# quiver-team/torch-quiver

Measured on AMD Instinct MI355X. Metric: train-sampled-edges/sec (GraphSAGE e2e step, ogbn-products-shaped synthetic), higher is better.
Workload: dtype fp32; 1 GPU; model=graphsage-3L-h256 ogbn-products, global_batch=1024, parallelism=dp1, sample_mode=GPU, cache=196M, cache_policy=device_replicate, placement=degree, overlap=True

## Files before the change

### csrc/gather_kernels.hip

```cpp
#include <cstdlib>

#include "qk_common.h"

namespace qk {

namespace {

constexpr int BLOCK = 256;

struct alignas(16) vec16 { uint64_t a, b; };

template <typename VecT, int SUB, bool SCATTER>
__global__ void __launch_bounds__(BLOCK)
copy_rows_kernel(GatherSpec spec, const int64_t* __restrict__ indices,
                 int64_t n, char* __restrict__ other,
                 const int64_t* __restrict__ n_dev,
                 const int64_t* __restrict__ order, int64_t order_n) {
    if (n_dev) n = min(n, *n_dev);
    const int sub_id = threadIdx.x / SUB;
    const int lane = threadIdx.x % SUB;
    const int rows_per_block = BLOCK / SUB;
    int64_t row = (int64_t)blockIdx.x * rows_per_block + sub_id;
    const int64_t stride = (int64_t)gridDim.x * rows_per_block;
    const int64_t nvec = spec.row_bytes / (int64_t)sizeof(VecT);

    for (; row < n; row += stride) {
        int64_t idx = indices[row];
        if (order) {
            if (idx < 0 || idx >= order_n) continue;
            idx = order[idx];
        }
        if (idx < 0) continue;
        int s = 0;
        while (s < spec.nshards && idx >= spec.ends[s]) ++s;
        if (s >= spec.nshards) continue;
        if (!((spec.access_mask >> s) & 1u)) continue;
        const int64_t start = (s == 0) ? 0 : spec.ends[s - 1];
        const char* shard_row =
            spec.ptrs[s] + (idx - start) * spec.row_bytes;
        char* io_row = other + row * spec.row_bytes;
        if (SCATTER) {
            VecT* dst = (VecT*)shard_row;
            const VecT* src = (const VecT*)io_row;
            for (int64_t j = lane; j < nvec; j += SUB) dst[j] = src[j];
        } else {
            const VecT* src = (const VecT*)shard_row;
            VecT* dst = (VecT*)io_row;
            for (int64_t j = lane; j < nvec; j += SUB) dst[j] = src[j];
        }
    }
}

inline int grid_for(int64_t work, int per_block, int max_blocks) {
    int64_t blocks = (work + per_block - 1) / per_block;
    if (blocks > max_blocks) blocks = max_blocks;
    if (blocks < 1) blocks = 1;
    return (int)blocks;
}

inline int gather_max_blocks(const GatherSpec& spec, bool overlapped) {
    static int env_cap = [] {
        const char* e = getenv("QUIVER_GATHER_BLOCKS");
        return e ? atoi(e) : 0;
    }();
    if (env_cap > 0) return env_cap;
    if (!spec.has_host_shard) return 2048;
    if (overlapped) return spec.row_bytes <= 256 ? 160 : 112;
    return 640;
}

template <typename VecT, bool SCATTER>
void dispatch_sub(hipStream_t s, const GatherSpec& spec,
                  const int64_t* indices, int64_t n, char* other,
                  const int64_t* n_dev, const int64_t* order,
                  int64_t order_n) {
    int64_t nvec = spec.row_bytes / (int64_t)sizeof(VecT);
    int sub = 4;
    while (sub < 64 && sub < nvec) sub *= 2;
    int grid = grid_for(n, BLOCK / sub,
                        gather_max_blocks(spec, n_dev != nullptr));
    switch (sub) {
#define QK_CASE(S)                                                          \
    case S:                                                                 \
        copy_rows_kernel<VecT, S, SCATTER><<<grid, BLOCK, 0, s>>>(          \
            spec, indices, n, other, n_dev, order, order_n);                \
        break;
        QK_CASE(4) QK_CASE(8) QK_CASE(16) QK_CASE(32) QK_CASE(64)
#undef QK_CASE
    }
    QK_CHECK_HIP(hipGetLastError());
}

template <bool SCATTER>
void copy_rows(hipStream_t s, const GatherSpec& spec, const int64_t* indices,
               int64_t n, char* other, const int64_t* n_dev,
               const int64_t* order, int64_t order_n) {
    if (n == 0 || spec.nshards == 0) return;
    if (spec.row_bytes % 16 == 0)
        dispatch_sub<vec16, SCATTER>(s, spec, indices, n, other, n_dev,
                                     order, order_n);
    else if (spec.row_bytes % 8 == 0)
        dispatch_sub<uint64_t, SCATTER>(s, spec, indices, n, other, n_dev,
                                        order, order_n);
    else if (spec.row_bytes % 4 == 0)
        dispatch_sub<uint32_t, SCATTER>(s, spec, indices, n, other, n_dev,
                                        order, order_n);
    else
        dispatch_sub<uint8_t, SCATTER>(s, spec, indices, n, other, n_dev,
                                       order, order_n);
}

}

void launch_gather(hipStream_t s, const GatherSpec& spec,
                   const int64_t* indices, int64_t n, char* out,
                   const int64_t* n_dev, const int64_t* order,
                   int64_t order_n) {
    copy_rows<false>(s, spec, indices, n, out, n_dev, order, order_n);
}

void launch_scatter(hipStream_t s, const GatherSpec& spec,
                    const int64_t* indices, int64_t n, const char* src) {
    copy_rows<true>(s, spec, indices, n, const_cast<char*>(src), nullptr,
                    nullptr, 0);
}

}
```

### csrc/module.cpp

```cpp
#include <torch/extension.h>

#include <ATen/Parallel.h>
#include <c10/hip/HIPCachingAllocator.h>
#include <c10/hip/HIPStream.h>
#include <hip/hip_runtime.h>
#include <rccl/rccl.h>

#include <algorithm>
#include <atomic>
#include <condition_variable>
#include <functional>
#include <mutex>
#include <thread>
#include <random>
#include <unordered_map>
#include <vector>

#include "qk_common.h"

namespace {

#define QK_CHECK_RCCL(expr)                                                   \
    do {                                                                      \
        ncclResult_t _r = (expr);                                             \
        if (_r != ncclSuccess) {                                              \
            throw std::runtime_error(std::string("RCCL error: ") +            \
                                     ncclGetErrorString(_r));                 \
        }                                                                     \
    } while (0)

inline hipStream_t current_stream() {
    return c10::hip::getCurrentHIPStream().stream();
}

inline int64_t next_pow2(int64_t x) {
    int64_t p = 64;
    while (p < x) p <<= 1;
    return p;
}

struct DeviceScope {
    int prev = -1;
    explicit DeviceScope(int dev) {
        QK_CHECK_HIP(hipGetDevice(&prev));
        if (dev != prev) QK_CHECK_HIP(hipSetDevice(dev));
    }
    ~DeviceScope() { (void)hipSetDevice(prev); }
};

void* register_host_chunked(void* p, size_t bytes,
                            std::vector<void*>& registered) {
    constexpr size_t kChunk = 1ull << 30;
    constexpr unsigned kFlags =
        hipHostRegisterMapped | hipHostRegisterPortable;
    auto devptr = [](void* hp) {
        void* dp = nullptr;
        QK_CHECK_HIP(hipHostGetDevicePointer(&dp, hp, 0));
        return dp;
    };
    char* base = (char*)p;
    std::vector<void*> regs;
    void* dp0 = nullptr;
    bool contiguous = true;
    for (size_t off = 0; off < bytes; off += kChunk) {
// ... 506 lines not shown
        }
        int64_t off = 0;
        for (int64_t i = 0; i < n; ++i)
            for (int64_t j = 0; j < cp[i]; ++j) rowp[off++] = i;
        TORCH_CHECK(off == m, "reindex: counts do not sum to neighbors");
        auto fr = torch::from_blob(frontier.data(),
                                   {(int64_t)frontier.size()},
                                   seeds.options())
                      .clone();
        return {fr, row, col};
    }

    int64_t node_count() const { return node_count_; }
    int64_t edge_count() const { return indices_.numel(); }

  private:
    torch::Tensor indptr_, indices_;
    int64_t node_count_;
};

struct ShardItem {
    void* dptr = nullptr;
    int64_t rows = 0;
    int device = -1;
    bool owned_hip = false;
    bool from_ipc = false;
    torch::Tensor keeper;
    std::vector<void*> host_regs;
};

class ShardTensorItem {
  public:
    int device = 0;
    int64_t rows = 0;
    std::vector<int64_t> row_shape;
    torch::Dtype dtype = torch::kFloat32;
    std::string handle;

    py::tuple share_ipc() {
        return py::make_tuple(device, py::bytes(handle), rows,
                              row_shape, (int)dtype);
    }
    static ShardTensorItem from_ipc(py::tuple t) {
        ShardTensorItem it;
        it.device = t[0].cast<int>();
        it.handle = t[1].cast<std::string>();
        it.rows = t[2].cast<int64_t>();
        it.row_shape = t[3].cast<std::vector<int64_t>>();
        it.dtype = (torch::Dtype)t[4].cast<int>();
        return it;
    }
};

class ShardTensor {
  public:
    explicit ShardTensor(int current_device) : device_(current_device) {}

    ~ShardTensor() {
        for (auto& s : shards_) {
            if (s.owned_hip) {
                DeviceScope g(s.device);
                (void)hipFree(s.dptr);
            } else if (s.from_ipc) {
                DeviceScope g(device_);
                (void)hipIpcCloseMemHandle(s.dptr);
            }
            for (void* r : s.host_regs) (void)hipHostUnregister(r);
        }
    }

    void append(torch::Tensor tensor, int target_device) {
        tensor = tensor.contiguous();
        TORCH_CHECK(tensor.dim() >= 1, "need at least 1-d tensor");
        init_row_meta(tensor);
        ShardItem item;
        item.rows = tensor.size(0);
        item.device = target_device;
        size_t bytes = (size_t)tensor.numel() * tensor.element_size();
        if (target_device >= 0) {
            DeviceScope g(target_device);
            QK_CHECK_HIP(hipMalloc(&item.dptr, bytes));
            if (tensor.device().is_cpu()) {
                QK_CHECK_HIP(hipMemcpy(item.dptr, tensor.data_ptr(), bytes,
                                       hipMemcpyHostToDevice));
            } else {
                QK_CHECK_HIP(hipMemcpy(item.dptr, tensor.data_ptr(), bytes,
                                       hipMemcpyDeviceToDevice));
            }
            item.owned_hip = true;
        } else {
            TORCH_CHECK(tensor.device().is_cpu(),
                        "host shard expects a CPU tensor");
            item.dptr = register_host_chunked(tensor.data_ptr(), bytes,
                                              item.host_regs);
            item.keeper = tensor;
        }
        shards_.push_back(std::move(item));
    }

    void append_from(const ShardTensor& other, int idx) {
        TORCH_CHECK(idx >= 0 && idx < (int)other.shards_.size(),
                    "append_from: no such shard");
        const ShardItem& s = other.shards_[idx];
        init_row_meta_from(other.row_shape_, other.dtype_);
        ShardItem item;
        item.dptr = s.dptr;
        item.rows = s.rows;
        item.device = s.device;
        item.keeper = s.keeper;
        shards_.push_back(std::move(item));
    }

    void append_item(const ShardTensorItem& it) {
        init_row_meta_from(it.row_shape, it.dtype);
        ShardItem item;
        item.rows = it.rows;
        item.device = it.device;
        item.from_ipc = true;
        DeviceScope g(device_);
        hipIpcMemHandle_t h;
        TORCH_CHECK(it.handle.size() == sizeof(h), "bad ipc handle");
        memcpy(&h, it.handle.data(), sizeof(h));
        QK_CHECK_HIP(hipIpcOpenMemHandle(&item.dptr, h,
                                         hipIpcMemLazyEnablePeerAccess));
        shards_.push_back(std::move(item));
    }

    std::vector<ShardTensorItem> share_ipc() {
        std::vector<ShardTensorItem> out;
        for (auto& s : shards_) {
            if (s.device < 0) continue;
            TORCH_CHECK(s.owned_hip,
                        "can only export shards this process allocated");
            ShardTensorItem it;
            it.device = s.device;
            it.rows = s.rows;
            it.row_shape = row_shape_;
            it.dtype = dtype_;
            hipIpcMemHandle_t h;
            DeviceScope g(s.device);
            QK_CHECK_HIP(hipIpcGetMemHandle(&h, s.dptr));
            it.handle.assign((char*)&h, sizeof(h));
            out.push_back(std::move(it));
        }
        return out;
    }

    torch::Tensor gather(torch::Tensor indices,
                         c10::optional<torch::Tensor> order) {
        return gather_impl(device_, indices, torch::Tensor(),
                           order.value_or(torch::Tensor()));
    }

    torch::Tensor gather_on(int dev, torch::Tensor indices) {
        return gather_impl(dev, indices, torch::Tensor(), torch::Tensor());
    }

    torch::Tensor gather_n(torch::Tensor indices, torch::Tensor n_dev,
                           c10::optional<torch::Tensor> order) {
        return gather_impl(device_, indices, n_dev,
                           order.value_or(torch::Tensor()));
    }

    torch::Tensor gather_impl(int dev, torch::Tensor indices,
                              torch::Tensor n_dev_t, torch::Tensor order_t) {
        DeviceScope g(dev);
        indices = indices.contiguous();
        TORCH_CHECK(indices.device().is_cuda(), "indices must be on GPU");
        TORCH_CHECK(indices.scalar_type() == torch::kInt64,
                    "indices must be int64");
        int64_t n = indices.numel();
        std::vector<int64_t> shape = {n};
        shape.insert(shape.end(), row_shape_.begin(), row_shape_.end());
        auto out = torch::empty(
            shape, torch::TensorOptions().dtype(dtype_).device(
                       torch::Device(torch::kCUDA, dev)));
        auto spec = build_spec(dev);
        auto cur = c10::hip::getCurrentHIPStream(dev);
        const int64_t* n_dev = n_dev_t.defined()
                                   ? n_dev_t.data_ptr<int64_t>()
                                   : nullptr;
        const int64_t* order = nullptr;
        int64_t order_n = 0;
        if (order_t.defined()) {
            TORCH_CHECK(order_t.is_cuda() && order_t.get_device() == dev &&
                            order_t.scalar_type() == torch::kInt64 &&
                            order_t.is_contiguous(),
                        "order must be a contiguous int64 tensor on the "
                        "executing device");
            order = order_t.data_ptr<int64_t>();
            order_n = order_t.numel();
        }

        uint32_t host_mask = 0;
        for (int i = 0; i < spec.nshards; ++i)
            if (shards_[i].device < 0) host_mask |= (1u << i);
        host_mask &= spec.access_mask;
        uint32_t dev_mask = spec.access_mask & ~host_mask;

        if (host_mask != 0 && dev_mask != 0 && staged_wanted(n)) {
            if (order) indices = order_t.index_select(0, indices);
            qk::GatherSpec ds = spec;
            ds.access_mask = dev_mask;
            ds.has_host_shard = false;
            qk::launch_gather(cur.stream(), ds, indices.data_ptr<int64_t>(),
                              n, (char*)out.data_ptr(), n_dev);
            gather_host_staged(dev, cur.stream(), indices, n, spec,
                               host_mask, out, n_dev);
        } else if (host_mask != 0 && dev_mask != 0) {
            qk::GatherSpec hs = spec;
            hs.access_mask = host_mask;
            hs.has_host_shard = true;
            qk::GatherSpec ds = spec;
            ds.access_mask = dev_mask;
            ds.has_host_shard = false;
            hipStreamCaptureStatus cs = hipStreamCaptureStatusNone;
            (void)hipStreamIsCapturing(cur.stream(), &cs);
            auto side = c10::hip::getCurrentHIPStream(dev);
            if (cs != hipStreamCaptureStatusNone) {
                side = c10::hip::getStreamFromPool(false, dev);
            } else {
                auto side_it = side_streams_.find(dev);
                if (side_it == side_streams_.end())
                    side_it = side_streams_
                                  .emplace(dev, c10::hip::getStreamFromPool(
                                                    false, dev))
                                  .first;
                side = side_it->second;
            }
            auto& ev = split_events_[dev];
            if (!ev.first) {
                QK_CHECK_HIP(hipEventCreateWithFlags(
                    &ev.first, hipEventDisableTiming));
                QK_CHECK_HIP(hipEventCreateWithFlags(
                    &ev.second, hipEventDisableTiming));
            }
            QK_CHECK_HIP(hipEventRecord(ev.first, cur.stream()));
            QK_CHECK_HIP(hipStreamWaitEvent(side.stream(), ev.first, 0));
            qk::launch_gather(cur.stream(), hs, indices.data_ptr<int64_t>(),
                              n, (char*)out.data_ptr(), n_dev, order,
                              order_n);
            qk::launch_gather(side.stream(), ds, indices.data_ptr<int64_t>(),
                              n, (char*)out.data_ptr(), n_dev, order,
                              order_n);
            QK_CHECK_HIP(hipEventRecord(ev.second, side.stream()));
            QK_CHECK_HIP(hipStreamWaitEvent(cur.stream(), ev.second, 0));
            if (cs == hipStreamCaptureStatusNone) {
                c10::hip::HIPCachingAllocator::recordStream(
                    out.storage().data_ptr(), side);
                c10::hip::HIPCachingAllocator::recordStream(
                    indices.storage().data_ptr(), side);
                if (order)
                    c10::hip::HIPCachingAllocator::recordStream(
                        order_t.storage().data_ptr(), side);
            }
        } else {
            qk::launch_gather(cur.stream(), spec,
                              indices.data_ptr<int64_t>(), n,
                              (char*)out.data_ptr(), n_dev, order, order_n);
        }
        return out;
    }

    void scatter_update(torch::Tensor indices, torch::Tensor src) {
        DeviceScope g(device_);
        indices = indices.contiguous();
        src = src.contiguous();
        auto spec = build_spec(device_);
        qk::launch_scatter(current_stream(), spec,
                           indices.data_ptr<int64_t>(), indices.numel(),
                           (const char*)src.data_ptr());
    }

    static bool staged_wanted(int64_t n) {
        static int mode = [] {
            const char* e = getenv("QUIVER_STAGED_GATHER");
            return e ? atoi(e) : -1;
        }();
        if (mode == 0) return false;
        if (mode == 1) return true;
        (void)n;
        return false;
    }

    void gather_host_staged(int dev, hipStream_t stream, torch::Tensor indices,
                            int64_t n, const qk::GatherSpec& spec,
                            uint32_t host_mask, torch::Tensor& out,
                            const int64_t* n_dev = nullptr) {
        const int64_t rb = row_bytes_;
        struct HostShard { int64_t beg, end; const char* base; };
        std::vector<HostShard> hosts;
        for (int s = 0; s < spec.nshards; ++s) {
            if (!((host_mask >> s) & 1u)) continue;
            int64_t beg = s == 0 ? 0 : spec.ends[s - 1];
            hosts.push_back({beg, spec.ends[s],
                             (const char*)shards_[s].keeper.data_ptr()});
        }
        if (hosts.empty()) return;

        auto pin_opts = torch::TensorOptions()
                            .dtype(torch::kUInt8)
                            .device(torch::kCPU)
                            .pinned_memory(true);
        if (!idx_pin_.defined() || idx_pin_.numel() < n * 8 + 8)
            idx_pin_ = torch::empty({n * 8 + 8}, pin_opts);
        QK_CHECK_HIP(hipMemcpyAsync(idx_pin_.data_ptr(),
                                    indices.data_ptr<int64_t>(), n * 8,
                                    hipMemcpyDeviceToHost, stream));
        int64_t* pinned_n =
            (int64_t*)((char*)idx_pin_.data_ptr() + idx_pin_.numel() - 8);
        if (n_dev)
            QK_CHECK_HIP(hipMemcpyAsync(pinned_n, n_dev, 8,
                                        hipMemcpyDeviceToHost, stream));
        QK_CHECK_HIP(hipStreamSynchronize(stream));
        if (n_dev) n = std::min(n, *pinned_n);
        const int64_t* idx = (const int64_t*)idx_pin_.data_ptr();

        const int64_t grain = 4096;
// ... 106 lines not shown
            TORCH_CHECK(rs == row_shape_ && dt == dtype_,
                        "all shards must share row shape and dtype");
            return;
        }
        row_shape_ = rs;
        dtype_ = dt;
        row_bytes_ = torch::elementSize(dt);
        for (auto d : rs) row_bytes_ *= d;
        row_shape_init_ = true;
    }

    qk::GatherSpec build_spec(int dev) const {
        TORCH_CHECK((int)shards_.size() <= qk::kMaxShards, "too many shards");
        qk::GatherSpec spec{};
        spec.nshards = (int)shards_.size();
        spec.row_bytes = row_bytes_;
        spec.access_mask = 0;
        spec.has_host_shard = false;
        int64_t acc = 0;
        DeviceScope g(dev);
        for (int i = 0; i < spec.nshards; ++i) {
            acc += shards_[i].rows;
            spec.ends[i] = acc;
            spec.ptrs[i] = (const char*)shards_[i].dptr;
            if (shards_[i].device < 0) spec.has_host_shard = true;
            bool ok = true;
            int sd = shards_[i].device;
            if (sd >= 0 && sd != dev) {
                int can = 0;
                QK_CHECK_HIP(hipDeviceCanAccessPeer(&can, dev, sd));
                if (can) {
                    hipError_t err = hipDeviceEnablePeerAccess(sd, 0);
                    if (err != hipSuccess &&
                        err != hipErrorPeerAccessAlreadyEnabled)
                        QK_CHECK_HIP(err);
                    (void)hipGetLastError();
                }
                ok = can || shards_[i].from_ipc;
            }
            if (ok) spec.access_mask |= (1u << i);
        }
        return spec;
    }

    int device_;
    std::vector<ShardItem> shards_;
    std::vector<int64_t> row_shape_;
    torch::Dtype dtype_ = torch::kFloat32;
    int64_t row_bytes_ = 0;
    bool row_shape_init_ = false;
    mutable std::unordered_map<int, std::pair<hipEvent_t, hipEvent_t>>
        split_events_;
    mutable std::unordered_map<int, c10::hip::HIPStream> side_streams_;
    torch::Tensor idx_pin_, pos_pin_, stage_pin_;
};


struct SegmentCall {
    const char* op;
    torch::Tensor feat, src, dst_ptr;
    int64_t n_dst = 0, dim;
    qk::Elem elem;
    DeviceScope scope;
    hipStream_t stream;

    SegmentCall(const char* op, const char* name, const torch::Tensor& f,
                bool fp32_only, const torch::Tensor* src_in,
                const torch::Tensor* dst_ptr_in)
        : op(op), feat(checked_rows(op, name, f, fp32_only)),
          dim(feat.size(1)),
          elem(feat.scalar_type() == torch::kBFloat16 ? qk::Elem::bf16
                                                      : qk::Elem::f32),
          scope(feat.get_device()),
          stream(c10::hip::getCurrentHIPStream(feat.get_device()).stream()) {
        if (src_in)
            src = arg("src", *src_in, torch::kInt64, {src_in->numel()});
        if (dst_ptr_in) {
            TORCH_CHECK(dst_ptr_in->numel() >= 1, op, ": dst_ptr is empty");
            dst_ptr = arg("dst_ptr", *dst_ptr_in, torch::kInt64,
                          {dst_ptr_in->numel()});
            n_dst = dst_ptr.numel() - 1;
        }
    }

    torch::Tensor arg(const char* name, const torch::Tensor& t,
                      torch::ScalarType dtype, at::IntArrayRef shape) const {
        TORCH_CHECK(t.device() == feat.device() && t.scalar_type() == dtype &&
                    t.sizes() == shape,
                    op, ": ", name, " must be ", dtype, " ", shape, " on ",
                    feat.device(), ", got ", t.scalar_type(), " ", t.sizes(),
                    " on ", t.device());
        return t.contiguous();
    }

    int chead(int64_t heads) const {
        TORCH_CHECK(heads > 0 && dim % heads == 0, op, ": feature dim ", dim,
                    " is not a multiple of heads ", heads);
        return (int)(dim / heads);
    }

    const int64_t* src_ptr() const { return src.data_ptr<int64_t>(); }
    const int64_t* dst_ptr_ptr() const { return dst_ptr.data_ptr<int64_t>(); }

  private:
    static torch::Tensor checked_rows(const char* op, const char* name,
                                      const torch::Tensor& t,
// ... 383 lines not shown
        .def("cal_neighbor_prob", &GpuSampler::cal_neighbor_prob,
             py::call_guard<py::gil_scoped_release>())
        .def("set_seed", &GpuSampler::set_seed)
        .def("node_count", &GpuSampler::node_count)
        .def("edge_count", &GpuSampler::edge_count)
        .def("device", &GpuSampler::device);

    m.def("device_quiver_from_csr_array",
          [](torch::Tensor indptr, torch::Tensor indices, torch::Tensor eid,
             int device, bool dma) {
              return new GpuSampler(indptr, indices, eid, device, dma);
          },
          py::return_value_policy::take_ownership);

    py::class_<CpuSampler>(m, "CPUQuiver")
        .def("sample_neighbor", &CpuSampler::sample_neighbor,
             py::call_guard<py::gil_scoped_release>())
        .def("reindex_single", &CpuSampler::reindex_single,
             py::call_guard<py::gil_scoped_release>())
        .def("node_count", &CpuSampler::node_count)
        .def("edge_count", &CpuSampler::edge_count);

    m.def("cpu_quiver_from_csr_array",
          [](torch::Tensor indptr, torch::Tensor indices) {
              return new CpuSampler(indptr, indices);
          },
          py::return_value_policy::take_ownership);

    py::class_<ShardTensorItem>(m, "ShardTensorItem")
        .def(py::init<>())
        .def("share_ipc", &ShardTensorItem::share_ipc)
        .def_static("from_ipc", &ShardTensorItem::from_ipc)
        .def_readwrite("device", &ShardTensorItem::device);

    py::class_<ShardTensor>(m, "ShardTensor")
        .def(py::init<int>())
        .def("append", &ShardTensor::append)
        .def("append_item", &ShardTensor::append_item)
        .def("append_from", &ShardTensor::append_from,
             "alias a shard owned by another same-process ShardTensor")
        .def("share_ipc", &ShardTensor::share_ipc)
        .def("__getitem__",
             [](ShardTensor& self, torch::Tensor indices) {
                 return self.gather(indices, c10::nullopt);
             },
             py::call_guard<py::gil_scoped_release>())
        .def("gather", &ShardTensor::gather, py::arg("indices"),
             py::arg("order") = py::none(),
             py::call_guard<py::gil_scoped_release>())
        .def("gather_on", &ShardTensor::gather_on,
             py::call_guard<py::gil_scoped_release>())
        .def("gather_n", &ShardTensor::gather_n, py::arg("indices"),
             py::arg("n_dev"), py::arg("order") = py::none(),
             py::call_guard<py::gil_scoped_release>())
        .def("access_mask_on", &ShardTensor::access_mask_on)
        .def("shard_ends", &ShardTensor::shard_ends)
        .def("scatter_update", &ShardTensor::scatter_update,
             py::call_guard<py::gil_scoped_release>())
        .def("shape", &ShardTensor::shape)
        .def("size", &ShardTensor::size)
        .def("device", &ShardTensor::device)
        .def("shard_count", &ShardTensor::shard_count)
        .def("shard_rows", &ShardTensor::shard_rows)
        .def("shard_devices", &ShardTensor::shard_devices);

    m.def("init_p2p", &init_p2p);
    m.def("can_device_access_peer", &can_device_access_peer);

    m.def("segment_mean_gather", &segment_mean_gather,
          py::call_guard<py::gil_scoped_release>());
    m.def("segment_mean_gather_backward", &segment_mean_gather_backward,
          py::call_guard<py::gil_scoped_release>());
    m.def("segment_mean_prefix_backward", &segment_mean_prefix_backward,
          py::arg("grad_agg"), py::arg("grad_self"), py::arg("src"),
          py::arg("dst_ptr"), py::arg("n_src"));
    m.def("segment_mean_lanes", &qk::segment_mean_lanes, py::arg("dim"),
          py::arg("bf16") = false);
    m.def("segment_mean_rows_in_flight", &qk::segment_mean_rows_in_flight);

    m.def("tall_gemm", &tall_gemm,
          "C[M,N] = A[M,K] @ B[K,N] (+bias), M huge, MFMA 32x32 tiles");
    m.def("gat_dots", &gat_dots,
          "fused per-head attention dots over a projected frontier");
    m.def("gat_dots_backward", &gat_dots_backward);
    m.def("gat_alpha", &gat_alpha,
          "fused GAT attention coefficients over dst-sorted edges");
    m.def("gat_alpha_backward", &gat_alpha_backward);
    m.def("segment_softmax", &segment_softmax,
          "numerically-stable softmax over dst-sorted edge segments");
    m.def("segment_softmax_backward", &segment_softmax_backward);
    m.def("segment_wsum", &segment_wsum,
          "weighted segment sum over dst-sorted edges (GAT aggregation)");
    m.def("segment_wsum_backward", &segment_wsum_backward);
    m.def("wgrad", &wgrad,
          "tall-skinny A^T@B (+ optional A column sums) via split-K atomics");
    m.def("create_nccl_id", &create_nccl_id);
    py::class_<RcclComm>(m, "NcclComm")
        .def(py::init<int, int, py::bytes>())
        .def("rank", &RcclComm::rank)
        .def("size", &RcclComm::size)
        .def("send", &RcclComm::send)
        .def("recv", &RcclComm::recv)
        .def("allreduce", &RcclComm::allreduce)
        .def("allgather", &RcclComm::allgather)
        .def("alltoall", &RcclComm::alltoall)
        .def("group_start", &RcclComm::group_start)
        .def("group_end", &RcclComm::group_end);
// ... 2 lines not shown
```

### csrc/qk_common.h

```cpp
#pragma once
#include <hip/hip_runtime.h>
#include <cstdint>
#include <stdexcept>
#include <string>

#define QK_CHECK_HIP(expr)                                                     \
    do {                                                                       \
        hipError_t _e = (expr);                                                \
        if (_e != hipSuccess) {                                                \
            throw std::runtime_error(std::string("HIP error at " __FILE__ ":") \
                                     + std::to_string(__LINE__) + ": "         \
                                     + hipGetErrorString(_e));                 \
        }                                                                      \
    } while (0)

namespace qk {

constexpr int kWaveSize = 64;


void launch_capped_degree(hipStream_t s, const int64_t* indptr,
                          const int64_t* seeds, int64_t n, int k,
                          int64_t* capped, const int64_t* n_dev = nullptr,
                          bool zero_extra_slot = false);
// ... 12 lines not shown

void launch_rng_bump(hipStream_t s, uint64_t* rng);

void launch_cal_next(hipStream_t s, const int64_t* indptr,
                     const int64_t* indices, const float* last, float* cur,
                     int64_t node_count, int k);


void launch_reindex_init(hipStream_t s, int64_t* keys, int32_t* pos,
                         int64_t capacity);
void launch_hash_insert(hipStream_t s, int64_t* keys, int32_t* pos,
                        int64_t capacity, const int64_t* seeds, int64_t n_seeds,
                        const int64_t* nbrs, int64_t n_nbrs,
                        const int64_t* n_seeds_dev = nullptr,
                        const int64_t* n_nbrs_dev = nullptr);
void launch_mark_first(hipStream_t s, const int64_t* keys, const int32_t* pos,
                       int64_t capacity, const int64_t* seeds, int64_t n_seeds,
                       const int64_t* nbrs, int64_t n_nbrs, int64_t* flags,
                       const int64_t* n_seeds_dev = nullptr,
                       const int64_t* n_nbrs_dev = nullptr);
void launch_compact_unique(hipStream_t s, const int64_t* keys, int32_t* local,
                           const int32_t* pos, int64_t capacity,
                           const int64_t* seeds, int64_t n_seeds,
                           const int64_t* nbrs, int64_t n_nbrs,
                           const int64_t* scanned_flags, const int64_t* flags,
                           int64_t* out_nodes,
                           const int64_t* n_seeds_dev = nullptr,
                           const int64_t* n_nbrs_dev = nullptr);
void launch_lookup_local(hipStream_t s, const int64_t* keys,
                         const int32_t* local, int64_t capacity,
                         const int64_t* nbrs, int64_t n_nbrs, int64_t* col_idx,
                         const int64_t* n_nbrs_dev = nullptr);
void launch_expand_rows(hipStream_t s, const int64_t* prefix,
                        const int64_t* counts, int64_t n_seeds,
                        int64_t* row_idx, const int64_t* n_dev = nullptr);


constexpr int kMaxShards = 16;

struct GatherSpec {
    const char* ptrs[kMaxShards];
    int64_t ends[kMaxShards];
    uint32_t access_mask;
    int nshards;
    int64_t row_bytes;
    bool has_host_shard;
};

void launch_gather(hipStream_t s, const GatherSpec& spec,
                   const int64_t* indices, int64_t n, char* out,
                   const int64_t* n_dev = nullptr,
                   const int64_t* order = nullptr, int64_t order_n = 0);

void launch_scatter(hipStream_t s, const GatherSpec& spec,
                    const int64_t* indices, int64_t n, const char* src);


void launch_tall_gemm(hipStream_t s, const float* A, const float* B,
                      const float* bias, float* C, int64_t M, int K, int N);


struct WgradPlan {
    int tm, tn;
    int64_t nchunks;
    int64_t k_chunk;
    int64_t ws_floats;
};
WgradPlan wgrad_plan(int64_t K, int M, int N);
void launch_wgrad(hipStream_t s, const float* A, const float* B, float* C,
                  float* bias_grad, int64_t K, int M, int N,
                  const WgradPlan& plan, float* ws);


enum class Elem { f32, bf16 };

void launch_segment_mean_fwd(hipStream_t s, Elem et, const void* x,
                             const int64_t* src, const int64_t* dst_ptr,
                             int64_t n_dst, int64_t dim, void* out);
void launch_segment_mean_bwd(hipStream_t s, Elem et, const void* grad_out,
                             const int64_t* src, const int64_t* dst_ptr,
                             int64_t n_dst, int64_t dim, void* grad_x);
int segment_mean_lanes(int64_t dim, bool bf16);
int segment_mean_rows_in_flight();
void launch_prefix_fill(hipStream_t s, const void* head, int64_t head_bytes,
                        int64_t total_bytes, void* out);

void launch_segment_wsum_fwd(hipStream_t s, Elem et, const void* x,
                             const float* w, const int64_t* src,
                             const int64_t* dst_ptr, int64_t n_dst, int heads,
                             int chead, void* out);
void launch_segment_wsum_bwd_x(hipStream_t s, Elem et, const void* grad_out,
                               const float* w, const int64_t* src,
                               const int64_t* dst_ptr, int64_t n_dst,
                               int heads, int chead, void* grad_x);
void launch_segment_wsum_bwd_w(hipStream_t s, Elem et, const void* grad_out,
                               const void* x, const int64_t* src,
                               const int64_t* dst_ptr, int64_t n_dst,
                               int heads, int chead, float* grad_w);

void launch_segment_softmax_fwd(hipStream_t s, const float* a,
                                const int64_t* dst_ptr, int64_t n_dst,
                                int heads, float* out);
void launch_segment_softmax_bwd(hipStream_t s, const float* grad_out,
                                const float* out, const int64_t* dst_ptr,
                                int64_t n_dst, int heads, float* grad_a);

// ... 22 lines not shown
```

### quiver/feature.py

```python
from typing import List

import numpy as np
import torch

from . import _ext
from .shard_tensor import ShardTensor, ShardTensorConfig
from .trace import trace_scope
from .utils import Topo, CSRTopo, hot_order, parse_size

__all__ = ["Feature", "DistFeature", "PartitionInfo", "DeviceConfig"]


class DeviceConfig:
    def __init__(self, gpu_parts, cpu_part):
        self.gpu_parts = gpu_parts
        self.cpu_part = cpu_part


class Feature(object):

    def __init__(self, rank: int, device_list: List[int],
                 device_cache_size=0, cache_policy="device_replicate",
                 csr_topo: CSRTopo = None):
        assert cache_policy in ["device_replicate", "p2p_clique_replicate"]
# ... 186 lines not shown
                appended = False
                for device in clique_devices:
                    cache_part = load_part(device_config.gpu_parts[device])
                    if cache_part.shape[0] > 0:
                        shard_tensor.append(cache_part, device)
                        appended = True
                if appended:
                    self.clique_tensor_list[clique_id] = shard_tensor

        if device_config.cpu_part is not None:
            cpu_part = device_config.cpu_part
            if isinstance(cpu_part, str):
                cpu_part = torch.from_numpy(np.load(cpu_part))
            elif np_array is not None and cpu_part.dim() == 1:
                cpu_part = torch.from_numpy(np_array[cpu_part.numpy()]).to(
                    dtype=torch.float32)
            self.cpu_part = cpu_part
            if self.cpu_part.numel() > 0:
                if self.cache_policy == "device_replicate":
                    shard_tensor = self.device_tensor_list.get(
                        self.rank, None) or ShardTensor(
                            self.rank, ShardTensorConfig({}))
                    shard_tensor.append(self.cpu_part, -1)
                    self.device_tensor_list[self.rank] = shard_tensor
                else:
                    clique_id = self.topo.get_clique_id(self.rank)
                    shard_tensor = self.clique_tensor_list.get(
                        clique_id, None) or ShardTensor(
                            self.rank, ShardTensorConfig({}))
                    shard_tensor.append(self.cpu_part, -1)
                    self.clique_tensor_list[clique_id] = shard_tensor

    def set_local_order(self, local_order):
        local_range = torch.arange(local_order.size(0), dtype=torch.int64,
                                   device=self.rank)
        self.feature_order = torch.zeros_like(local_range)
        self.feature_order[local_order.to(self.rank)] = local_range

    def set_mmap_file(self, path, disk_map):
        self.lazy_init_from_ipc_handle()
        self.mmap_handle_ = np.load(path, mmap_mode="r")
        self.disk_map = disk_map.to(self.rank)

    def read_mmap(self, ids):
        ids = ids.cpu().numpy()
        res = torch.from_numpy(self.mmap_handle_[ids])
        return res.to(device=self.rank, dtype=torch.float32)

    def _shard_tensor(self):
        if self.cache_policy == "device_replicate":
            return self.device_tensor_list[self.rank]
        return self.clique_tensor_list[self.topo.get_clique_id(self.rank)]

    def gather_raw(self, node_idx, n_dev):
        self.lazy_init_from_ipc_handle()
        if self.mmap_handle_ is not None:
            raise RuntimeError("gather_raw does not support the disk tier")
        node_idx = node_idx.to(self.rank)
        return self._shard_tensor().gather_n(node_idx, n_dev,
                                             self.feature_order)

    def __getitem__(self, node_idx: torch.Tensor):
        self.lazy_init_from_ipc_handle()
        node_idx = node_idx.to(self.rank)
        if self.mmap_handle_ is None:
            with trace_scope("feature.gather"):
                return self._shard_tensor().gather(node_idx,
                                                   self.feature_order)
        num_nodes = node_idx.size(0)
        disk_index = self.disk_map[node_idx]
        node_range = torch.arange(num_nodes, device=node_idx.device,
                                  dtype=torch.int64)
        disk_mask = disk_index < 0
        mem_mask = disk_index >= 0
        disk_ids = torch.masked_select(node_idx, disk_mask)
        disk_pos = torch.masked_select(node_range, disk_mask)
        mem_ids = torch.masked_select(node_idx, mem_mask)
        mem_pos = torch.masked_select(node_range, mem_mask)
        local_mem_ids = self.disk_map[mem_ids]
        disk_res = self.read_mmap(disk_ids)
        mem_res = self._shard_tensor()[local_mem_ids]
        res = torch.zeros((num_nodes, self.size(1)), device=node_idx.device,
                          dtype=mem_res.dtype)
        res[disk_pos] = disk_res.to(res.dtype)
        res[mem_pos] = mem_res
        return res

    def size(self, dim: int):
        self.lazy_init_from_ipc_handle()
        return self._shard_tensor().size(dim)

    def dim(self):
        return len(self.shape)

    @property
    def shape(self):
        self.lazy_init_from_ipc_handle()
        return self._shard_tensor().shape

    @property
    def ipc_handle(self):
        return self.ipc_handle_

    @ipc_handle.setter
    def ipc_handle(self, ipc_handle):
        self.ipc_handle_ = ipc_handle

    def share_ipc(self):
        self.cpu_part.share_memory_()
        gpu_ipc_handle_dict = {}
        if self.cache_policy == "device_replicate":
            for device in self.device_tensor_list:
                gpu_ipc_handle_dict[device] = \
# ... 130 lines not shown
```

### quiver/loader.py

```python
import os
from collections import deque

import torch

from .pyg.sage_sampler import DST_PTR_ATTR

__all__ = ["TrainingPrefetcher"]


class _GraphedChain:

    def __init__(self, sampler, feature, seeds_proto, stream, depth):
        self.batch_size = seeds_proto.numel()
        self.slots = []
        self.turn = 0
        device = sampler.device
        H = len(sampler.sizes)
        for _ in range(depth + 1):
            static_seeds = seeds_proto.to(device).clone()
            sizes_pin = torch.empty(2 * H, dtype=torch.int64,
                                    pin_memory=True)
            g = torch.cuda.CUDAGraph()
            with torch.cuda.stream(stream):
                with torch.cuda.graph(g, stream=stream):
                    raw, sizes_dev, ptrs = sampler.quiver.sample_hops_raw(
                        static_seeds, sampler.sizes)
                    x_ub = None
                    if feature is not None:
                        n_dev = sizes_dev[2 * H - 1:2 * H]
                        x_ub = feature.gather_raw(raw[H - 1][0], n_dev)
            tok = (static_seeds, raw, sizes_dev, sizes_pin, ptrs)
            self.slots.append((static_seeds, g, tok, x_ub))

    def run(self, seeds):
        static_seeds, g, tok, x_ub = self.slots[self.turn]
        self.turn = (self.turn + 1) % len(self.slots)
        static_seeds.copy_(seeds, non_blocking=True)
        g.replay()
        tok[3].copy_(tok[2], non_blocking=True)
        return tok, x_ub


class TrainingPrefetcher:
    def __init__(self, sampler, feature, seed_batches, depth=2, device=None,
                 num_streams=1):
        self.sampler = sampler
        self.feature = feature
        self.seed_batches = seed_batches
        self.depth = max(1, depth, num_streams)
        self.num_streams = max(1, num_streams)
        self.device = device if device is not None \
            else torch.cuda.current_device()

    def _can_chain_async(self):
        if not hasattr(self.sampler, "sample_async"):
            return False
        if getattr(self.sampler, "mode", None) not in ("GPU", "UVA"):
            return False
        if getattr(self.sampler, "sort_frontier", False):
            return False
        if self.feature is not None:
            if not hasattr(self.feature, "gather_raw"):
                return False
            if getattr(self.feature, "mmap_handle_", None) is not None:
                return False
            try:
                st = self.feature._shard_tensor()
                if st._inaccessible_ranges():
                    return False
            except Exception:
                pass
        return True

    def __iter__(self):
        cur = torch.cuda.current_stream(self.device)
        sides = [torch.cuda.Stream(self.device, priority=-1)
                 for _ in range(self.num_streams)]
        it = iter(self.seed_batches)
        pending = deque()
        main_evs = deque()
        chain_async = [self._can_chain_async()]
        want_graph = (chain_async[0] and self.num_streams == 1
                      and os.environ.get("QUIVER_HIPGRAPH", "0") == "1")
        graphed = [None]
        produced = [0]
        rr = [0]

        def produce():
            try:
                seeds = next(it)
            except StopIteration:
                return False
            idx = rr[0] % len(sides)
            rr[0] += 1
            if chain_async[0] and want_graph and graphed[0] is None \
                    and produced[0] >= 1:
                try:
                    graphed[0] = _GraphedChain(self.sampler, self.feature,
                                               seeds, sides[idx],
                                               self.depth)
                except Exception as e:
                    import warnings
                    warnings.warn("TrainingPrefetcher: hipGraph capture "
                                  f"failed ({e}); running uncaptured",
                                  RuntimeWarning)
                    graphed[0] = False
                    sides[idx] = torch.cuda.Stream(self.device,
                                                   priority=-1)
            side = sides[idx]
            if want_graph:
                ev_main = torch.cuda.Event()
                ev_main.record(cur)
                main_evs.append(ev_main)
                if len(main_evs) > 2:
                    main_evs.popleft()
            with torch.cuda.stream(side):
                if chain_async[0] and isinstance(graphed[0], _GraphedChain) \
                        and seeds.numel() == graphed[0].batch_size:
                    side.wait_event(main_evs[0])
                    try:
                        tok, x_ub = graphed[0].run(seeds)
                        ev = torch.cuda.Event()
                        ev.record(side)
                        pending.append(("gtok", tok, x_ub, ev))
                        produced[0] += 1
                        return True
                    except RuntimeError as e:
                        import warnings
                        warnings.warn("TrainingPrefetcher: hipGraph replay "
                                      f"failed ({e}); running uncaptured",
                                      RuntimeWarning)
                        graphed[0] = False
                if chain_async[0]:
                    try:
                        tok = self.sampler.sample_async(seeds)
                        x_ub = None
                        if self.feature is not None:
                            raw, sizes_dev = tok[1], tok[2]
                            n_dev = sizes_dev[2 * len(raw) - 1:2 * len(raw)]
                            x_ub = self.feature.gather_raw(raw[-1][0], n_dev)
                        ev = torch.cuda.Event()
                        ev.record(side)
                        pending.append(("tok", tok, x_ub, ev))
                        produced[0] += 1
                        return True
                    except RuntimeError as e:
                        import warnings
                        warnings.warn(
                            "TrainingPrefetcher: zero-sync chain disabled "
                            f"after: {e}", RuntimeWarning)
                        chain_async[0] = False
                n_id, bs, adjs = self.sampler.sample(seeds)
                x = self.feature[n_id] if self.feature is not None else None
                ev = torch.cuda.Event()
                ev.record(side)
            pending.append(("done", (n_id, bs, adjs), x, ev))
            return True

        for _ in range(self.depth):
            if not produce():
                break
        while pending:
            kind, payload, x, ev = pending.popleft()
            cur.wait_event(ev)
            if kind in ("tok", "gtok"):
                ev.synchronize()
                n_id, bs, adjs = self.sampler.sample_finalize(payload)
                if x is not None:
                    x = x[:n_id.size(0)]
            else:
                n_id, bs, adjs = payload
            if kind == "gtok":
                pass
            else:
                if kind == "tok":
                    for f_ub, e_ub in payload[1]:
                        e_ub.record_stream(cur)
                    for p_ub in payload[4]:
                        p_ub.record_stream(cur)
                n_id.record_stream(cur)
                for adj in adjs:
                    adj.edge_index.record_stream(cur)
                    ptr = getattr(adj.edge_index, DST_PTR_ATTR, None)
                    if ptr is not None:
                        ptr.record_stream(cur)
                if x is not None:
                    x.record_stream(cur)
            yield n_id, bs, adjs, x
            produce()
```

### quiver/shard_tensor.py

```python
from typing import Dict, NamedTuple

import torch

from . import _ext
from .utils import parse_size


class Offset(NamedTuple):
    start: int
    end: int


class ShardTensorConfig:

    def __init__(self, device_memory_budget: Dict[int, object]):
        self.tensor_offset_device: Dict[int, Offset] = {}
        self.device_memory_budget = {
            d: parse_size(b) for d, b in (device_memory_budget or {}).items()
        }

    @property
    def device_list(self):
        return list(self.device_memory_budget.keys())

# ... 8 lines not shown
    def partition(self, tensor, memory_budget):
        row_bytes = tensor[0].numel() * tensor.element_size()
        return parse_size(memory_budget) // row_bytes

    def append(self, tensor, device):
        start = self.shard_tensor.size(0) if self.shard_tensor.shard_count() else 0
        self.shard_tensor.append(tensor, device)
        end = start + tensor.size(0)
        if device >= 0:
            self.shard_tensor_config.tensor_offset_device[device] = Offset(
                start, end)
        if device == -1:
            self.cpu_tensor = tensor

    def from_cpu_tensor(self, tensor):
        cur_pos = 0
        for device_id, budget in self.shard_tensor_config.device_memory_budget.items():
            if cur_pos >= tensor.shape[0]:
                break
            size = min(self.partition(tensor, budget),
                       tensor.shape[0] - cur_pos)
            if size <= 0:
                continue
            self.append(tensor[cur_pos:cur_pos + size], device_id)
            cur_pos += size
        if cur_pos < tensor.shape[0]:
            self.append(tensor[cur_pos:], -1)

    def _inaccessible_ranges(self):
        if not torch.cuda.is_available():
            return []
        mask = self.shard_tensor.access_mask_on(self.current_device)
        ends = self.shard_tensor.shard_ends()
        devices = self.shard_tensor.shard_devices()
        out = []
        start = 0
        for i, end in enumerate(ends):
            if not (mask >> i) & 1:
                out.append((start, end, devices[i]))
            start = end
        return out

    def collect_device(self, input_orders, nodes, inter_device, start, end,
                       wait_results):
        mask = (nodes >= start) & (nodes < end)
        request_nodes = torch.masked_select(nodes, mask)
        if request_nodes.numel() == 0:
            return
        part_orders = torch.masked_select(input_orders, mask)
        request_nodes = request_nodes.to(inter_device)
        result = self.shard_tensor.gather_on(inter_device, request_nodes)
        wait_results.append((part_orders, result.to(self.current_device)))

    def gather_n(self, nodes, n_dev, order=None):
        if self._inaccessible_ranges():
            raise RuntimeError("gather_n: some shards need the cross-clique "
                               "pass; use __getitem__")
        nodes = nodes.to(self.current_device)
        return self.shard_tensor.gather_n(nodes, n_dev, order)

    def __getitem__(self, nodes):
        return self.gather(nodes)

    def gather(self, nodes, order=None):
        nodes = nodes.to(self.current_device)
        missing = self._inaccessible_ranges()
        if missing and order is not None:
            nodes = order[nodes]
            order = None
        feature = self.shard_tensor.gather(nodes, order)
        if missing:
            input_orders = torch.arange(nodes.size(0), dtype=torch.long,
                                        device=nodes.device)
            wait_results = []
            for start, end, dev in missing:
                self.collect_device(input_orders, nodes, dev, start, end,
                                    wait_results)
            for orders, result in wait_results:
                feature[orders] = result
        return feature

    @property
    def shape(self):
        return torch.Size(self.shard_tensor.shape())

    @property
    def device(self):
        return self.current_device

    def size(self, dim):
        return self.shard_tensor.size(dim)

    def share_ipc(self):
        items = [it.share_ipc() for it in self.shard_tensor.share_ipc()]
        if self.cpu_tensor is not None:
            self.cpu_tensor.share_memory_()
        return items, self.cpu_tensor, self.current_device

    def from_ipc_handle(self, gpu_ipc_list, cpu_tensor):
        for item in gpu_ipc_list:
            self.shard_tensor.append_item(_ext.ShardTensorItem.from_ipc(item))
        if cpu_tensor is not None:
            self.shard_tensor.append(cpu_tensor, -1)
            self.cpu_tensor = cpu_tensor

    @classmethod
    def new_from_share_ipc(cls, ipc_handles, current_device):
        gpu_ipc_list, cpu_tensor, _ = ipc_handles
        st = cls(current_device, ShardTensorConfig({}))
        st.from_ipc_handle(gpu_ipc_list, cpu_tensor)
        return st
```

Baseline: 188.6 million edges/s.

## Reuse host-tier feature rows from the previous two gather outputs on device

Adds a per-row table, sized to the host-resident part of the feature tensor, that records which recent gather output (and which row in it) last fetched each host row. A new gather kernel copies such rows from one of the last two device-resident output tensors instead of reading them over the host link. The training prefetcher enables this by default when the host row count is small enough relative to the frontier. The ring slots are invalidated on append and scatter_update. In exchange it keeps up to two old outputs alive, adds a table read and write per row, and makes each gather wait on the previous reuse gathers' completion events, which may reduce overlap between batches.

```diff
diff --git a/csrc/gather_kernels.hip b/csrc/gather_kernels.hip
--- a/csrc/gather_kernels.hip
+++ b/csrc/gather_kernels.hip
@@ -51,6 +51,67 @@
     }
 }
 
+template <typename VecT, int SUB>
+__global__ void __launch_bounds__(BLOCK)
+copy_rows_reuse_kernel(GatherSpec spec, GatherReuse ru,
+                       const int64_t* __restrict__ indices, int64_t n,
+                       char* __restrict__ out,
+                       const int64_t* __restrict__ n_dev,
+                       const int64_t* __restrict__ order, int64_t order_n) {
+    n = min(n, *n_dev);
+    const int sub_id = threadIdx.x / SUB;
+    const int lane = threadIdx.x % SUB;
+    const int rows_per_block = BLOCK / SUB;
+    int64_t row = (int64_t)blockIdx.x * rows_per_block + sub_id;
+    const int64_t stride = (int64_t)gridDim.x * rows_per_block;
+    const int64_t nvec = spec.row_bytes / (int64_t)sizeof(VecT);
+
+    auto copy_row = [&](int64_t r, int64_t idx, uint64_t e) {
+        if (idx < 0) return;
+        const char* base = nullptr;
+        int64_t start = 0;
+        for (int i = 0; i < spec.nshards; ++i) {
+            const int64_t lo = (i == 0) ? 0 : spec.ends[i - 1];
+            if (idx >= lo && idx < spec.ends[i] &&
+                ((spec.access_mask >> i) & 1u)) {
+                base = spec.ptrs[i];
+                start = lo;
+            }
+        }
+        if (!base) return;
+        const char* src_row = base + (idx - start) * spec.row_bytes;
+
+        const int64_t t = idx - ru.row_base;
+        const bool tracked = t >= 0 && t < ru.rows;
+        if (tracked) {
+            const uint32_t e_seq = (uint32_t)(e >> 32);
+            const int64_t e_row = (int64_t)(e & 0xffffffffu);
+            const uint32_t age = ru.seq - e_seq;
+            if (e_seq != 0 && age >= 1 && age <= (uint32_t)kReuseWindow) {
+                const char* p = age == 1 ? ru.src[0] : ru.src[1];
+                const int64_t p_rows =
+                    age == 1 ? ru.src_rows[0] : ru.src_rows[1];
+                if (p && e_row < p_rows) src_row = p + e_row * spec.row_bytes;
+            }
+        }
+        const VecT* src = (const VecT*)src_row;
+        VecT* dst = (VecT*)(out + r * spec.row_bytes);
+        for (int64_t j = lane; j < nvec; j += SUB) dst[j] = src[j];
+        if (tracked && lane == 0)
+            ru.table[t] = ((uint64_t)ru.seq << 32) | (uint64_t)r;
+    };
+
+    for (; row < n; row += stride) {
+        int64_t idx = indices[row];
+        if (order) {
+            if (idx < 0 || idx >= order_n) continue;
+            idx = order[idx];
+        }
+        const int64_t t = idx - ru.row_base;
+        copy_row(row, idx, (t >= 0 && t < ru.rows) ? ru.table[t] : 0);
+    }
+}
+
 inline int grid_for(int64_t work, int per_block, int max_blocks) {
     int64_t blocks = (work + per_block - 1) / per_block;
     if (blocks > max_blocks) blocks = max_blocks;
@@ -73,7 +134,7 @@
 void dispatch_sub(hipStream_t s, const GatherSpec& spec,
                   const int64_t* indices, int64_t n, char* other,
                   const int64_t* n_dev, const int64_t* order,
-                  int64_t order_n) {
+                  int64_t order_n, const GatherReuse* ru = nullptr) {
     int64_t nvec = spec.row_bytes / (int64_t)sizeof(VecT);
     int sub = 4;
     while (sub < 64 && sub < nvec) sub *= 2;
@@ -82,6 +143,13 @@
     switch (sub) {
 #define QK_CASE(S)                                                          \
     case S:                                                                 \
+        if constexpr (!SCATTER) {                                           \
+            if (ru) {                                                       \
+                copy_rows_reuse_kernel<VecT, S><<<grid, BLOCK, 0, s>>>(     \
+                    spec, *ru, indices, n, other, n_dev, order, order_n);   \
+                break;                                                      \
+            }                                                               \
+        }                                                                   \
         copy_rows_kernel<VecT, S, SCATTER><<<grid, BLOCK, 0, s>>>(          \
             spec, indices, n, other, n_dev, order, order_n);                \
         break;
@@ -94,20 +162,21 @@
 template <bool SCATTER>
 void copy_rows(hipStream_t s, const GatherSpec& spec, const int64_t* indices,
                int64_t n, char* other, const int64_t* n_dev,
-               const int64_t* order, int64_t order_n) {
+               const int64_t* order, int64_t order_n,
+               const GatherReuse* ru = nullptr) {
     if (n == 0 || spec.nshards == 0) return;
     if (spec.row_bytes % 16 == 0)
         dispatch_sub<vec16, SCATTER>(s, spec, indices, n, other, n_dev,
-                                     order, order_n);
+                                     order, order_n, ru);
     else if (spec.row_bytes % 8 == 0)
         dispatch_sub<uint64_t, SCATTER>(s, spec, indices, n, other, n_dev,
-                                        order, order_n);
+                                        order, order_n, ru);
     else if (spec.row_bytes % 4 == 0)
         dispatch_sub<uint32_t, SCATTER>(s, spec, indices, n, other, n_dev,
-                                        order, order_n);
+                                        order, order_n, ru);
     else
         dispatch_sub<uint8_t, SCATTER>(s, spec, indices, n, other, n_dev,
-                                       order, order_n);
+                                       order, order_n, ru);
 }
 
 }
@@ -119,6 +188,17 @@
     copy_rows<false>(s, spec, indices, n, out, n_dev, order, order_n);
 }
 
+void launch_gather_reuse(hipStream_t s, const GatherSpec& spec,
+                         const int64_t* indices, int64_t n, char* out,
+                         const int64_t* n_dev, const int64_t* order,
+                         int64_t order_n, const GatherReuse& ru) {
+    if (!n_dev || !ru.table || ru.seq == 0 || n > (int64_t)UINT32_MAX)
+        throw std::runtime_error(
+            "launch_gather_reuse: needs a device-side count, a table, a "
+            "sequence number >= 1 and at most 2^32-1 rows");
+    copy_rows<false>(s, spec, indices, n, out, n_dev, order, order_n, &ru);
+}
+
 void launch_scatter(hipStream_t s, const GatherSpec& spec,
                     const int64_t* indices, int64_t n, const char* src) {
     copy_rows<true>(s, spec, indices, n, const_cast<char*>(src), nullptr,
diff --git a/csrc/module.cpp b/csrc/module.cpp
--- a/csrc/module.cpp
+++ b/csrc/module.cpp
@@ -9,7 +9,9 @@
 #include <algorithm>
 #include <atomic>
 #include <condition_variable>
+#include <climits>
 #include <functional>
+#include <memory>
 #include <mutex>
 #include <thread>
 #include <random>
@@ -622,6 +624,24 @@
     }
 };
 
+struct ReuseSlot {
+    torch::Tensor out;
+    uint32_t seq = 0;
+    hipEvent_t done = nullptr;
+};
+
+struct ReuseState {
+    torch::Tensor table;
+    int64_t row_base = 0, rows = 0;
+    uint32_t next_seq = 1;
+    uint32_t floor = 0;
+    ReuseSlot ring[qk::kReuseWindow];
+    ~ReuseState() {
+        for (auto& slot : ring)
+            if (slot.done) (void)hipEventDestroy(slot.done);
+    }
+};
+
 class ShardTensor {
   public:
     explicit ShardTensor(int current_device) : device_(current_device) {}
@@ -643,6 +663,7 @@
         tensor = tensor.contiguous();
         TORCH_CHECK(tensor.dim() >= 1, "need at least 1-d tensor");
         init_row_meta(tensor);
+        drop_reuse_sources();
         ShardItem item;
         item.rows = tensor.size(0);
         item.device = target_device;
@@ -727,13 +748,21 @@
     }
 
     torch::Tensor gather_n(torch::Tensor indices, torch::Tensor n_dev,
-                           c10::optional<torch::Tensor> order) {
+                           c10::optional<torch::Tensor> order, bool reuse) {
         return gather_impl(device_, indices, n_dev,
-                           order.value_or(torch::Tensor()));
+                           order.value_or(torch::Tensor()), reuse);
+    }
+
+    void drop_reuse_sources() {
+        std::lock_guard<std::mutex> lk(reuse_mu_);
+        if (!reuse_) return;
+        reuse_->floor = reuse_->next_seq - 1;
+        for (auto& slot : reuse_->ring) slot.out = torch::Tensor();
     }
 
     torch::Tensor gather_impl(int dev, torch::Tensor indices,
-                              torch::Tensor n_dev_t, torch::Tensor order_t) {
+                              torch::Tensor n_dev_t, torch::Tensor order_t,
+                              bool reuse_wanted = false) {
         DeviceScope g(dev);
         indices = indices.contiguous();
         TORCH_CHECK(indices.device().is_cuda(), "indices must be on GPU");
@@ -807,14 +836,31 @@
             }
             QK_CHECK_HIP(hipEventRecord(ev.first, cur.stream()));
             QK_CHECK_HIP(hipStreamWaitEvent(side.stream(), ev.first, 0));
-            qk::launch_gather(cur.stream(), hs, indices.data_ptr<int64_t>(),
-                              n, (char*)out.data_ptr(), n_dev, order,
-                              order_n);
+            const bool reuse = reuse_wanted && reuse_enabled() &&
+                               dev == device_ && n_dev != nullptr &&
+                               n > 0 && cs == hipStreamCaptureStatusNone;
+            std::unique_lock<std::mutex> reuse_lk;
+            ReuseSlot* slot = nullptr;
+            if (reuse) {
+                reuse_lk = std::unique_lock<std::mutex>(reuse_mu_);
+                slot = launch_host_reuse(cur, hs, host_mask, indices, n, out,
+                                         n_dev, order, order_n);
+            } else {
+                qk::launch_gather(cur.stream(), hs,
+                                  indices.data_ptr<int64_t>(), n,
+                                  (char*)out.data_ptr(), n_dev, order,
+                                  order_n);
+            }
             qk::launch_gather(side.stream(), ds, indices.data_ptr<int64_t>(),
                               n, (char*)out.data_ptr(), n_dev, order,
                               order_n);
             QK_CHECK_HIP(hipEventRecord(ev.second, side.stream()));
             QK_CHECK_HIP(hipStreamWaitEvent(cur.stream(), ev.second, 0));
+            if (slot) {
+                QK_CHECK_HIP(hipEventRecord(slot->done, cur.stream()));
+                slot->out = out;
+                reuse_lk.unlock();
+            }
             if (cs == hipStreamCaptureStatusNone) {
                 c10::hip::HIPCachingAllocator::recordStream(
                     out.storage().data_ptr(), side);
@@ -832,8 +878,86 @@
         return out;
     }
 
+    static bool reuse_enabled() {
+        static bool on = [] {
+            const char* e = getenv("QUIVER_GATHER_REUSE");
+            return !(e && atoi(e) == 0);
+        }();
+        return on;
+    }
+
+    ReuseSlot* launch_host_reuse(c10::hip::HIPStream cur,
+                                 const qk::GatherSpec& hs, uint32_t host_mask,
+                                 const torch::Tensor& indices, int64_t n,
+                                 const torch::Tensor& out,
+                                 const int64_t* n_dev, const int64_t* order,
+                                 int64_t order_n) {
+        constexpr int W = qk::kReuseWindow;
+        TORCH_CHECK(n <= (int64_t)UINT32_MAX,
+                    "gather_n(reuse=True): more than 2^32-1 rows");
+        int64_t lo = INT64_MAX, hi = 0;
+        for (int s = 0; s < hs.nshards; ++s) {
+            if (!((host_mask >> s) & 1u)) continue;
+            lo = std::min(lo, s == 0 ? (int64_t)0 : hs.ends[s - 1]);
+            hi = std::max(hi, hs.ends[s]);
+        }
+        if (!reuse_ || reuse_->row_base != lo || reuse_->rows != hi - lo) {
+            auto st = std::make_unique<ReuseState>();
+            st->table = torch::zeros(
+                {hi - lo}, torch::TensorOptions().dtype(torch::kInt64).device(
+                               out.device()));
+            st->row_base = lo;
+            st->rows = hi - lo;
+            reuse_ = std::move(st);
+        }
+        ReuseState& st = *reuse_;
+        for (auto& slot : st.ring)
+            if (slot.seq != 0 && slot.done)
+                QK_CHECK_HIP(hipStreamWaitEvent(cur.stream(), slot.done, 0));
+        if (st.next_seq == UINT32_MAX) {
+            QK_CHECK_HIP(hipMemsetAsync(st.table.data_ptr(), 0,
+                                        (size_t)st.rows * 8, cur.stream()));
+            for (auto& slot : st.ring) {
+                slot.out = torch::Tensor();
+                slot.seq = 0;
+            }
+            st.next_seq = 1;
+            st.floor = 0;
+        }
+        const uint32_t seq = st.next_seq++;
+
+        qk::GatherReuse ru{};
+        ru.table = (uint64_t*)st.table.data_ptr<int64_t>();
+        ru.row_base = st.row_base;
+        ru.rows = st.rows;
+        ru.seq = seq;
+        for (int k = 0; k < W; ++k) {
+            const int64_t want = (int64_t)seq - 1 - k;
+            if (want < 1 || want <= (int64_t)st.floor) continue;
+            ReuseSlot& src = st.ring[want % W];
+            if (src.seq != (uint32_t)want || !src.out.defined()) continue;
+            ru.src[k] = (const char*)src.out.data_ptr();
+            ru.src_rows[k] = src.out.size(0);
+            c10::hip::HIPCachingAllocator::recordStream(
+                src.out.storage().data_ptr(), cur);
+        }
+        c10::hip::HIPCachingAllocator::recordStream(
+            st.table.storage().data_ptr(), cur);
+        qk::launch_gather_reuse(cur.stream(), hs, indices.data_ptr<int64_t>(),
+                                n, (char*)out.data_ptr(), n_dev, order,
+                                order_n, ru);
+        ReuseSlot& slot = st.ring[seq % W];
+        if (!slot.done)
+            QK_CHECK_HIP(hipEventCreateWithFlags(&slot.done,
+                                                 hipEventDisableTiming));
+        slot.seq = seq;
+        slot.out = torch::Tensor();
+        return &slot;
+    }
+
     void scatter_update(torch::Tensor indices, torch::Tensor src) {
         DeviceScope g(device_);
+        drop_reuse_sources();
         indices = indices.contiguous();
         src = src.contiguous();
         auto spec = build_spec(device_);
@@ -1046,6 +1170,8 @@
     mutable std::unordered_map<int, std::pair<hipEvent_t, hipEvent_t>>
         split_events_;
     mutable std::unordered_map<int, c10::hip::HIPStream> side_streams_;
+    std::mutex reuse_mu_;
+    std::unique_ptr<ReuseState> reuse_;
     torch::Tensor idx_pin_, pos_pin_, stage_pin_;
 };
 
@@ -1535,7 +1661,10 @@
              py::call_guard<py::gil_scoped_release>())
         .def("gather_n", &ShardTensor::gather_n, py::arg("indices"),
              py::arg("n_dev"), py::arg("order") = py::none(),
+             py::arg("reuse") = false,
              py::call_guard<py::gil_scoped_release>())
+        .def("drop_reuse_sources", &ShardTensor::drop_reuse_sources,
+             "no earlier gather output is a row-reuse source from here on")
         .def("access_mask_on", &ShardTensor::access_mask_on)
         .def("shard_ends", &ShardTensor::shard_ends)
         .def("scatter_update", &ShardTensor::scatter_update,
diff --git a/csrc/qk_common.h b/csrc/qk_common.h
--- a/csrc/qk_common.h
+++ b/csrc/qk_common.h
@@ -88,6 +88,20 @@
                    const int64_t* n_dev = nullptr,
                    const int64_t* order = nullptr, int64_t order_n = 0);
 
+constexpr int kReuseWindow = 2;
+struct GatherReuse {
+    uint64_t* table;
+    int64_t row_base, rows;
+    uint32_t seq;
+    const char* src[kReuseWindow];
+    int64_t src_rows[kReuseWindow];
+};
+
+void launch_gather_reuse(hipStream_t s, const GatherSpec& spec,
+                         const int64_t* indices, int64_t n, char* out,
+                         const int64_t* n_dev, const int64_t* order,
+                         int64_t order_n, const GatherReuse& ru);
+
 void launch_scatter(hipStream_t s, const GatherSpec& spec,
                     const int64_t* indices, int64_t n, const char* src);
 
diff --git a/quiver/feature.py b/quiver/feature.py
--- a/quiver/feature.py
+++ b/quiver/feature.py
@@ -262,13 +262,13 @@
             return self.device_tensor_list[self.rank]
         return self.clique_tensor_list[self.topo.get_clique_id(self.rank)]
 
-    def gather_raw(self, node_idx, n_dev):
+    def gather_raw(self, node_idx, n_dev, reuse=False):
         self.lazy_init_from_ipc_handle()
         if self.mmap_handle_ is not None:
             raise RuntimeError("gather_raw does not support the disk tier")
         node_idx = node_idx.to(self.rank)
         return self._shard_tensor().gather_n(node_idx, n_dev,
-                                             self.feature_order)
+                                             self.feature_order, reuse)
 
     def __getitem__(self, node_idx: torch.Tensor):
         self.lazy_init_from_ipc_handle()
diff --git a/quiver/loader.py b/quiver/loader.py
--- a/quiver/loader.py
+++ b/quiver/loader.py
@@ -42,8 +42,13 @@
 
 
 class TrainingPrefetcher:
+
+    REUSE_MAX_HOST_ROWS_PER_SLOT = 16
+
     def __init__(self, sampler, feature, seed_batches, depth=2, device=None,
-                 num_streams=1):
+                 num_streams=1, reuse_rows=True):
+        self.reuse_rows = bool(reuse_rows)
+        self._host_rows = None
         self.sampler = sampler
         self.feature = feature
         self.seed_batches = seed_batches
@@ -72,7 +77,37 @@
                 pass
         return True
 
+    def _gather_raw(self, frontier, n_dev):
+        if not self.reuse_rows:
+            return self.feature.gather_raw(frontier, n_dev)
+        if self._host_rows is None:
+            self.feature.lazy_init_from_ipc_handle()
+            st = self.feature._shard_tensor().shard_tensor
+            self._host_rows = sum(
+                r for r, d in zip(st.shard_rows(), st.shard_devices())
+                if d < 0)
+        reuse = (self._host_rows
+                 <= self.REUSE_MAX_HOST_ROWS_PER_SLOT * frontier.numel())
+        return self.feature.gather_raw(frontier, n_dev, reuse=reuse)
+
+    def _drop_reuse_sources(self):
+        if not (self.reuse_rows and hasattr(self.feature, "_shard_tensor")):
+            return
+        try:
+            st = self.feature._shard_tensor()
+        except Exception:
+            return
+        if hasattr(st, "drop_reuse_sources"):
+            st.drop_reuse_sources()
+
     def __iter__(self):
+        self._drop_reuse_sources()
+        try:
+            yield from self._iterate()
+        finally:
+            self._drop_reuse_sources()
+
+    def _iterate(self):
         cur = torch.cuda.current_stream(self.device)
         sides = [torch.cuda.Stream(self.device, priority=-1)
                  for _ in range(self.num_streams)]
@@ -138,7 +173,7 @@
                         if self.feature is not None:
                             raw, sizes_dev = tok[1], tok[2]
                             n_dev = sizes_dev[2 * len(raw) - 1:2 * len(raw)]
-                            x_ub = self.feature.gather_raw(raw[-1][0], n_dev)
+                            x_ub = self._gather_raw(raw[-1][0], n_dev)
                         ev = torch.cuda.Event()
                         ev.record(side)
                         pending.append(("tok", tok, x_ub, ev))
diff --git a/quiver/shard_tensor.py b/quiver/shard_tensor.py
--- a/quiver/shard_tensor.py
+++ b/quiver/shard_tensor.py
@@ -84,12 +84,15 @@
         result = self.shard_tensor.gather_on(inter_device, request_nodes)
         wait_results.append((part_orders, result.to(self.current_device)))
 
-    def gather_n(self, nodes, n_dev, order=None):
+    def gather_n(self, nodes, n_dev, order=None, reuse=False):
         if self._inaccessible_ranges():
             raise RuntimeError("gather_n: some shards need the cross-clique "
                                "pass; use __getitem__")
         nodes = nodes.to(self.current_device)
-        return self.shard_tensor.gather_n(nodes, n_dev, order)
+        return self.shard_tensor.gather_n(nodes, n_dev, order, reuse)
+
+    def drop_reuse_sources(self):
+        self.shard_tensor.drop_reuse_sources()
 
     def __getitem__(self, nodes):
         return self.gather(nodes)
```

Result: faster. 213.6 million edges/s (median of 6 runs) (+13.3%).
